# RomanBresson/KAGNN

Hardware: AMD Instinct MI355X
Metric: edges/sec KAN-GIN fwd+bwd, hidden=64 grid=5, 1M-node synthetic; HBM % peak (higher is better)
Workload: dtype f32 (fp16 hi/lo split operands, fp32 accumulate)

## Files before the change

### kagnn_amd/csrc/kan_sparse_fwd.hip

```cpp
#include "split_common.h"

namespace kagnn {

typedef _Float16 f16x16 __attribute__((ext_vector_type(16)));

constexpr int kSpCF = 64;
constexpr int kSpOutBlk = 64;
constexpr int kSpOutBlkWide = 128;
constexpr int kSpSteps = kSpCF / 4;
__host__ __device__ inline size_t sparse_fwd_chunk_bytes(int OT) {
    return (size_t)kSpSteps * OT * 2 * 2048 + (size_t)(kSpCF / 16) * OT * 2 * 1024;
}

bool kan_sparse_fwd_ok(int in, int out, int G, int K) { return K == 3 && G + K <= 16; }
__host__ __device__ inline int sp_sh(int C) { return C > 8 ? 1 : 0; }

static size_t sp_chunks_bytes(int inv, int ob) { return (size_t)cdiv(inv, kSpCF) * sparse_fwd_chunk_bytes(cdiv(ob, 32)); }
static size_t sp_blk_bytes(int in, int inv, int ob) { return kHdrBytes + sp_chunks_bytes(inv, ob) + (((size_t)ob * in * 4 + 255) & ~(size_t)255); }
static bool sp_wide_enabled() {
    static const bool on = [] { const char* e = getenv("KAGNN_FWD_WIDE"); return !(e && e[0] == '0'); }();
    return on;
}
static int sp_out_blk(int inv , int out) {
    return (sp_wide_enabled() && out % kSpOutBlkWide == 0 && inv > 32) ? kSpOutBlkWide : kSpOutBlk;
// ... 334 lines not shown
                    for (int st = 1; st < AEP; st <<= 1)
#pragma unroll
                        for (int k = 0; k < AEP; k += 2 * st) {
                            acc[g][h][k].x += acc[g][h][k + st].x; acc[g][h][k].y += acc[g][h][k + st].y;
                            acc[g][h][k].z += acc[g][h][k + st].z; acc[g][h][k].w += acc[g][h][k + st].w;
                        }
                    o[h] = make_float4(fmaf(sw, self[g][h].x, acc[g][h][0].x), fmaf(sw, self[g][h].y, acc[g][h][0].y),
                                       fmaf(sw, self[g][h].z, acc[g][h][0].z), fmaf(sw, self[g][h].w, acc[g][h][0].w));
                }
            }
            const int f0 = kg * HF + 8 * g;
            if (l0[g]) *reinterpret_cast<float4*>(ag.h0 + row * ag.ldh + f0) = o[0];
            if (l1[g]) *reinterpret_cast<float4*>(ag.h0 + row * ag.ldh + f0 + 4) = o[1];
            if (!l0[g]) o[0] = make_float4(0.f, 0.f, 0.f, 0.f);
            if (!l1[g]) o[1] = make_float4(0.f, 0.f, 0.f, 0.f);
            xa[g][0] = o[0].x; xa[g][1] = o[0].y; xa[g][2] = o[0].z; xa[g][3] = o[0].w;
            xa[g][4] = o[1].x; xa[g][5] = o[1].y; xa[g][6] = o[1].z; xa[g][7] = o[1].w;
        }
    };
    auto place1 = [&](const u32x4& e, unsigned h0, unsigned h1, unsigned l0, unsigned l1, unsigned& hi0, unsigned& hi1,
                      unsigned& lo0, unsigned& lo1) {
        hi0 = __builtin_amdgcn_perm(h1, h0, e[0]); hi1 = __builtin_amdgcn_perm(h1, h0, e[1]);
        lo0 = __builtin_amdgcn_perm(l1, l0, e[0]); lo1 = __builtin_amdgcn_perm(l1, l0, e[1]);
    };

    const int ng_live = HF / 8;
    (void)ng_live;
    float mom_n = 0.0f;
    float* s_momw = reinterpret_cast<float*>(s_w + BUF_BYTES) + wave * (OT * 64);
    if constexpr (MOM) {
#pragma unroll
        for (int t = 0; t < OT; ++t) s_momw[64 * t + lane] = 0.0f;
    }
    float xn[8];
    float xa[AGG >= 0 ? AGRP : 1][8];
    if constexpr (AGG >= 0) {
        gather_tile((long)blockIdx.x * ROWS, xa);
#pragma unroll
        for (int j = 0; j < 8; ++j) xn[j] = xa[0][j];
    } else load8((long)blockIdx.x * ROWS, ch_begin, 0, xn);
    for (long tile = blockIdx.x; tile * ROWS < N; tile += gridDim.x) {
        const long row0 = tile * ROWS + wave * 32;
        f32x16 acc[OT], acc_b[MERGED ? 1 : OT];
#pragma unroll
        for (int t = 0; t < OT; ++t)
#pragma unroll
            for (int i = 0; i < 16; ++i) { acc[t][i] = 0.0f; if constexpr (!MERGED) acc_b[t][i] = 0.0f; }

        for (int ch = ch_begin; ch < ch_end; ++ch) {
#pragma unroll
            for (int g = 0; g < NG; ++g) {
                if (g >= ng_live) continue;
                const int q = g / GPP, gq = g % GPP;
                const unsigned char* hb = s_w + (q & 1) * HALF_BYTES;
                if (!resident && gq == 0) {
                    lds_dma_wait();
                    __syncthreads();
#ifndef KAGNN_ABLATE_FWD_NO_REFILL
                    if (q + 1 < PPC) dma_half(ch, q + 1);
                    else if (ch + 1 < ch_end) dma_half(ch + 1, 0);
                    else if ((tile + gridDim.x) * ROWS < N) dma_half(ch_begin, 0);
#endif
                }
                float xv[8];
#pragma unroll
                for (int j = 0; j < 8; ++j) xv[j] = xn[j];
                if constexpr (AGG >= 0) {
                    if (g + 1 < ng_live) {
#pragma unroll
                        for (int j = 0; j < 8; ++j) xn[j] = xa[AGRP - 1][j];
                    } else {
                        gather_tile((tile + gridDim.x) * ROWS, xa);
#pragma unroll
                        for (int j = 0; j < 8; ++j) xn[j] = xa[0][j];
                    }
                } else if (g + 1 < ng_live) load8(tile * ROWS, ch, g + 1, xn);
                else if (ch + 1 < ch_end) load8(tile * ROWS, ch + 1, 0, xn);
                else load8((tile + gridDim.x) * ROWS, ch_begin, 0, xn);

                u32x4 ahi, alo, bw[4 * OT];
                int aidx;
                auto prep_reads = [&](int s, u32x4& e0, u32x4& e1, float& u0, float& u1, u32x4 (&w)[4 * OT]) {
                    unsigned o0, o1;
                    frag3_index<false>(xv[2 * s], f3geo, u0, o0);
                    if constexpr (SH) { u1 = u0; o1 = o0 + 512u; }
                    else frag3_index<false>(xv[2 * s + 1], f3geo, u1, o1);
                    e0 = *reinterpret_cast<const u32x4*>(reinterpret_cast<const unsigned char*>(s_tbl) + o0);
                    e1 = *reinterpret_cast<const u32x4*>(reinterpret_cast<const unsigned char*>(s_tbl) + o1);
                    if constexpr (MERGED) return;
                    const unsigned char* wp = hb + (size_t)((4 * gq + s) * OT) * 2 * 2048 + lane * 16;
#pragma unroll
                    for (int i = 0; i < 2 * OT; ++i) {
                        if (HALF && (i & 1)) continue;
                        w[2 * i] = *reinterpret_cast<const u32x4*>(wp + i * 2048);
                        w[2 * i + 1] = *reinterpret_cast<const u32x4*>(wp + i * 2048 + 1024);
                    }
                };
                auto read_w = [&](int s, u32x4 (&w)[4 * OT]) {
                    const unsigned char* wp = hb + (size_t)((4 * gq + s) * OT) * 2 * 2048 + lane * 16;
#pragma unroll
                    for (int i = 0; i < 2 * OT; ++i) {
                        w[2 * i] = *reinterpret_cast<const u32x4*>(wp + i * 2048);
                        w[2 * i + 1] = *reinterpret_cast<const u32x4*>(wp + i * 2048 + 1024);
                    }
                };
                auto build = [&](int s, const u32x4& e0, const u32x4& e1, float u0, float u1, u32x4& hi, u32x4& lo, int& idx) {
                    unsigned a0, a1, a2, a3, b0 = 0, b1 = 0, b2 = 0, b3 = 0, h0, h1, l0, l1;
#ifdef KAGNN_ABLATE_FWD_NO_EXPAND
                    hi = u32x4{__float_as_uint(u0), __float_as_uint(u1), e0[0], e1[0]};
                    lo = u32x4{e0[1], e1[1], __float_as_uint(u1), __float_as_uint(u0)};
                    idx = (int)(e0[2] | (e1[2] << 8));
// ... 120 lines not shown
                }
                if constexpr (!MERGED) {
                if (!big) {

                    const unsigned char* wp = hb + HALF_SPL + (size_t)(gq * OT) * 2 * 1024 + lane * 16;
#pragma unroll
                    for (int t = 0; t < OT; ++t) {
                        f32x16& ab = MERGED ? acc[t] : acc_b[MERGED ? 0 : t];
                        const u32x4 wh = *reinterpret_cast<const u32x4*>(wp + (t * 2 + 0) * 1024);
                        ab = mfma_f16(sh_hi, wh, ab);
                        if constexpr (!HALF) {
                            const u32x4 wl = *reinterpret_cast<const u32x4*>(wp + (t * 2 + 1) * 1024);
                            ab = mfma_f16(sh_hi, wl, ab);
                            ab = mfma_f16(sh_lo, wh, ab);
                        }
                    }
                } else {
                    const int f0 = ch * CF + kg * HF + 8 * g;
#pragma unroll
                    for (int j = 0; j < 8; ++j) {
#pragma unroll
                        for (int t = 0; t < OT; ++t) {
                            const int o = 32 * t + r;
                            const int fr = SH ? (f0 + j) >> 1 : f0 + j;
                            const float w = (o < out && fr < in && !(SH && (j & 1))) ? base_w[(long)o * in + fr] : 0.0f;
                            f32x16& ab = MERGED ? acc[t] : acc_b[MERGED ? 0 : t];
                            ab = __builtin_amdgcn_mfma_f32_32x32x2f32(sv[j] * (MERGED ? 0.0009765625f : 0.0625f), w * wsc16, ab, 0, 0, 0);
                        }
                    }
                }
                }
            }
        }
        const GBuf yb = gbuf_at(y, N, ldy, out, tile * ROWS);
        const long rows_here = min(32L, N - row0);
        const float mom_nt = (float)max(rows_here, 1L), mom_rnt = __builtin_amdgcn_rcpf(mom_nt);
        const float mom_w = mom_nt * __builtin_amdgcn_rcpf(mom_n + mom_nt), mom_nw = mom_n * mom_w;
#pragma unroll
        for (int t = 0; t < OT; ++t) {
            const int col = 32 * t + r;
            const unsigned base = (unsigned)(wave * 32 + 4 * kg) * ldy4 + col * 4;
            float v[16];
#pragma unroll
            for (int i = 0; i < 16; ++i) v[i] = MERGED ? acc[t][i] * post : fmaf(acc[t][i], post, acc_b[MERGED ? 0 : t][i] * post_b);
            if (col < out) {
#pragma unroll
                for (int i = 0; i < 16; ++i)
                    gst_s(yb, base, (unsigned)((i & 3) + 8 * (i >> 2)) * ldy4, v[i]);
            }
            if constexpr (MOM) {
                float sm = 0.0f, q = 0.0f, mt;
                if (rows_here >= 32) {
#pragma unroll
                    for (int i = 0; i < 16; ++i) sm += v[i];
                    sm += __shfl_xor(sm, 32);
                    mt = sm * mom_rnt;
#pragma unroll
                    for (int i = 0; i < 16; ++i) { const float d = v[i] - mt; q = fmaf(d, d, q); }
                } else {
#pragma unroll
                    for (int i = 0; i < 16; ++i) sm += (4 * kg + (i & 3) + 8 * (i >> 2) < rows_here) ? v[i] : 0.0f;
                    sm += __shfl_xor(sm, 32);
                    mt = sm * mom_rnt;
#pragma unroll
                    for (int i = 0; i < 16; ++i) {
                        const float d = (4 * kg + (i & 3) + 8 * (i >> 2) < rows_here) ? v[i] - mt : 0.0f;
                        q = fmaf(d, d, q);
// ... 373 lines not shown
```

### kagnn_amd/csrc/kan_split_bwd.hip

```cpp
#include <type_traits>
#include "split_common.h"

namespace kagnn {

int kan_dw_reduce(const float* slab, long NS, long per_slab, float* gcat, hipStream_t st);

int kan_dw_unpack(const float* gcat, int in, int out, int C, long inP, long outP, const float* sw,
                  const float* sc, float* g_bw, float* g_sw, float* g_sc, hipStream_t st);


bool kan_split_dx_ok(int in, int out, int G, int K) { return K >= 0 && K <= 4 && G + K <= 16; }
static inline int vshift(int C) { return C > 8 ? 1 : 0; }

static size_t dx_blk_bytes(int inv , int ob) {
    return kHdrBytes + (size_t)cdiv(inv, 16) * kCTmax * dx_q2(ob) * 2 * 1024;
}
bool kan_dx_w2_ok(int in, int out, int C, int K) { return K == 3 && C > 8 && C <= 16 && out <= kOutBlk; }
static int dx_inv(int in, int out, int C, int K) { return kan_dx_w2_ok(in, out, C, K) ? 32 * cdiv(in, 16) : (in << vshift(C)); }

size_t kan_split_pack_dx_bytes(int in, int out, int C, int K) {
    return (size_t)cdiv(out, kOutBlk) * dx_blk_bytes(dx_inv(in, out, C, K), min(out, kOutBlk));
}

__global__ void split_pack_dx_kernel(const float* __restrict__ bw, const float* __restrict__ sw,
// ... 86 lines not shown
        const unsigned char* src = gw + (size_t)ft0 * FT_BYTES;
        const int nblk = nft * (FT_BYTES / 1024);
        if constexpr (HALF) {
            for (int blk = 2 * wave; blk < nblk; blk += 16)
                lds_dma_1k(src + (size_t)blk * 1024 + lane * 16, __builtin_amdgcn_readfirstlane(lds_w + blk * 1024));
        } else
        for (int blk = wave; blk < nblk; blk += 8)
            lds_dma_1k(src + (size_t)blk * 1024 + lane * 16, __builtin_amdgcn_readfirstlane(lds_w + blk * 1024));
        lds_dma_wait();
    };
    const int ft_begin = blockIdx.y * ft_per_block, ft_end = min(FT, ft_begin + ft_per_block);
    if (resident) stage(ft_begin, ft_end - ft_begin);
    __syncthreads();
    const bool pingpong = (PP == 2) && resident;
    SplineGeom geom{}; FastGeom fgeo{};
    const int li = lane & 15, kg = lane >> 4;
    const int win = li & sh;
    float ca[8] = {};
    if constexpr (K == 0) {
        float c0[8], c1[8];
        rbf_centers(rb, c0, 0); rbf_centers(rb, c1, sh);
#pragma unroll
        for (int g = 0; g < 8; ++g) ca[g] = win ? c1[g] : c0[g];
    }
    if constexpr (K > 0) { geom = geom_from_knots(s_knots, nknots); fgeo = fast_geom(s_knots, nknots); }
    const bool ln_on = (K == 0) && rb.ln_w != nullptr;
    const bool al4 = ((ldgy & 3) == 0) && ((reinterpret_cast<uintptr_t>(gy) & 15) == 0);
    const unsigned ldx4 = (unsigned)ldx * 4u, ldgy4 = (unsigned)ldgy * 4u, ldgx4 = (unsigned)ldgx * gxes;
    const unsigned gy_ro = (unsigned)(wave * 32 + li) * ldgy4;
    const unsigned x_rb = (unsigned)(wave * 32 + 4 * kg) * ldx4;
    const unsigned gx_rb = (unsigned)(wave * 32 + 4 * kg) * ldgx4;
    const unsigned gz_rb = (unsigned)(wave * 32 + 4 * kg) * (unsigned)in * 4u;

    auto load_gy = [&](long tile, float (&raw)[2][Q2][8]) {
        const GBuf gyb = gbuf_at(gy, N, ldgy, out, tile * 256);
#pragma unroll
        for (int rt = 0; rt < 2; ++rt) {
            const unsigned ro = gy_ro + kg * 32;
            const unsigned so = (unsigned)(16 * rt) * ldgy4;
#pragma unroll
            for (int q = 0; q < Q2; ++q) {
                if (al4 && 32 * Q2 == out) {
                    gld4_s(gyb, ro, so + 128 * q, raw[rt][q]);
                    gld4_s(gyb, ro, so + 128 * q + 16, raw[rt][q] + 4);
                } else if (al4 && (out & 7) == 0) {
                    const unsigned rq = gy_ro + (unsigned)min(32 * q + 8 * kg, out - 8) * 4u;
                    gld4_s(gyb, rq, so, raw[rt][q]);
                    gld4_s(gyb, rq, so + 16, raw[rt][q] + 4);
                } else {
                    const int o0 = 32 * q + 8 * kg;
#pragma unroll
                    for (int j = 0; j < 8; ++j) raw[rt][q][j] = gld_s(gyb, gy_ro + min(o0 + j, out - 1) * 4, so);
                }
            }
        }
        if constexpr (BNB) {
            const GBuf yb = gbuf_at(bnb.y, N, bnb.ldy, out, tile * 256), ob = gbuf_at(bnb.gy_out, N, bnb.ldo, out, tile * 256);
            const unsigned ldy4 = (unsigned)bnb.ldy * 4u, ldo4 = (unsigned)bnb.ldo * 4u;
            const unsigned yro = (unsigned)(wave * 32 + li) * ldy4 + kg * 32, oro = (unsigned)(wave * 32 + li) * ldo4 + kg * 32;
#pragma unroll
            for (int q = 0; q < Q2; ++q) {
                float cm[8], cA[8], cB[8], cC[8];
                const float* t0 = bnb.tab + 32 * q + 8 * kg;
#pragma unroll
                for (int h = 0; h < 2; ++h) {
                    const float4 a = *reinterpret_cast<const float4*>(t0 + 4 * h), b = *reinterpret_cast<const float4*>(t0 + bnb.ldt + 4 * h);
                    const float4 c = *reinterpret_cast<const float4*>(t0 + 2 * bnb.ldt + 4 * h), d = *reinterpret_cast<const float4*>(t0 + 3 * bnb.ldt + 4 * h);
                    cm[4 * h] = a.x; cm[4 * h + 1] = a.y; cm[4 * h + 2] = a.z; cm[4 * h + 3] = a.w;
                    cA[4 * h] = b.x; cA[4 * h + 1] = b.y; cA[4 * h + 2] = b.z; cA[4 * h + 3] = b.w;
                    cB[4 * h] = c.x; cB[4 * h + 1] = c.y; cB[4 * h + 2] = c.z; cB[4 * h + 3] = c.w;
                    cC[4 * h] = d.x; cC[4 * h + 1] = d.y; cC[4 * h + 2] = d.z; cC[4 * h + 3] = d.w;
                }
#pragma unroll
                for (int rt = 0; rt < 2; ++rt) {
                    float yv[8];
                    gld4_s(yb, yro, (unsigned)(16 * rt) * ldy4 + 128 * q, yv);
                    gld4_s(yb, yro, (unsigned)(16 * rt) * ldy4 + 128 * q + 16, yv + 4);
#pragma unroll
                    for (int j = 0; j < 8; ++j) raw[rt][q][j] = bn_bwd_value(raw[rt][q][j], yv[j], cm[j], cA[j], cB[j], cC[j]);
                    if (blockIdx.y == 0) {
                        gst4_s(ob, oro, (unsigned)(16 * rt) * ldo4 + 128 * q, raw[rt][q]);
                        gst4_s(ob, oro, (unsigned)(16 * rt) * ldo4 + 128 * q + 16, raw[rt][q] + 4);
                    }
                }
            }
        }
    };
    u32x4 ahi[2][Q2], alo[2][Q2];
    float rinv[2][4];
    auto split_gy = [&](const float (&raw)[2][Q2][8]) {
#pragma unroll
        for (int rt = 0; rt < 2; ++rt) {
            float mx = 0.0f;
#pragma unroll
            for (int q = 0; q < Q2; ++q)
#pragma unroll
                for (int j = 0; j < 8; ++j) mx = fmaxf(mx, fabsf(raw[rt][q][j]));
            mx = fmaxf(mx, __shfl_xor(mx, 16));
            mx = fmaxf(mx, __shfl_xor(mx, 32));
            const int rexp = exp_for_max(mx);
            const float sc = ldexpf(1.0f, 10 - rexp);
#pragma unroll
            for (int q = 0; q < Q2; ++q) {
                float v[8];
#pragma unroll
                for (int j = 0; j < 8; ++j) v[j] = raw[rt][q][j] * sc;
                if constexpr (HALF) round_f16x2(v, ahi[rt][q]);
                else split_f16x2_asm(v, ahi[rt][q], alo[rt][q]);
            }
            const float mine = ldexpf(1.0f, e_w + rexp - 10);
#pragma unroll
            for (int reg = 0; reg < 4; ++reg) rinv[rt][reg] = __shfl(mine, 4 * kg + reg);
        }
    };
    float mu[2][4], rs[2][4];
    auto load_stats = [&](long tile) {
        if (ln_on) {
            const long row0 = tile * 256 + wave * 32;
#pragma unroll
            for (int rt = 0; rt < 2; ++rt)
#pragma unroll
                for (int reg = 0; reg < 4; ++reg) {
                    const long rc = min(row0 + 16 * rt + 4 * kg + reg, N - 1);
                    mu[rt][reg] = rb.stats[2 * rc]; rs[rt][reg] = rb.stats[2 * rc + 1];
                }
        }
    };

    float* s_stat = reinterpret_cast<float*>(s_w + (size_t)(ft_end - ft_begin) * FT_BYTES) + wave * 128;
    if constexpr (XST) { s_stat[lane] = 0.0f; s_stat[64 + lane] = 0.0f; }
    float graw[2][Q2][8];
    long tile = blockIdx.x;
    if (!XST && tile * 256 >= N) return;
    if (!XST || tile * 256 < N) {
    load_gy(tile, graw);
    load_stats(tile);
    split_gy(graw);
    if (PP >= 1 && (tile + gridDim.x) * 256 < N) load_gy(tile + gridDim.x, graw);
    }
    if (pingpong && wave >= 4) __builtin_amdgcn_s_barrier();

    for (; tile * 256 < N; tile += gridDim.x) {
        const bool more = (tile + gridDim.x) * 256 < N;
        if (PP == 0 && tile != (long)blockIdx.x) {
            load_gy(tile, graw);
            load_stats(tile);
            split_gy(graw);
        }
        const GBuf gzb = gbuf_at(rb.gz, N, in, in, tile * 256);
        const GBuf xb = gbuf_at(x, N, ldx, in, tile * 256), gxb = gbuf_at_es(gx, N, ldgx, in, tile * 256, (int)gxes);

        for (int ft = ft_begin; ft < ft_end; ++ft) {
            if (!resident) {
                __syncthreads();
                stage(ft, 1);
                __syncthreads();
            }
            const unsigned char* wft = s_w + (size_t)(resident ? ft - ft_begin : 0) * FT_BYTES + lane * 16;
            const int f = 16 * ft + li;
            const int fr = f >> sh;
            const unsigned fcol = (unsigned)min(fr, in - 1) * 4u;
            const unsigned gx_ro = gx_rb + (unsigned)min(fr, in - 1) * gxes, gz_ro = gz_rb + fcol;
            float gam = 1.0f, bet = 0.0f;
            if (ln_on) { gam = rb.ln_w[min(fr, in - 1)]; bet = rb.ln_b[min(fr, in - 1)]; }
            float xa = 1.0f, xs = 0.0f;
            if constexpr (XAFF) { xa = rb.x_affine[min(fr, in - 1)]; xs = rb.x_affine[in + min(fr, in - 1)]; }
            float st_m = 0.0f, st_q = 0.0f, st_g = 0.0f, st_gx = 0.0f;
            if constexpr (XST) { st_m = rb.st_mean[min(fr, in - 1)]; st_q = rb.st_rstd[min(fr, in - 1)]; }
            float xq[2][4];
#pragma unroll
            for (int rt = 0; rt < 2; ++rt)
#pragma unroll
                for (int reg = 0; reg < 4; ++reg) {
                    xq[rt][reg] = gld_s(xb, x_rb + fcol, (unsigned)(16 * rt + reg) * ldx4);
                }
            f32x4 D[kCTmax][2];
#pragma unroll
            for (int c = 0; c < kCTmax; ++c) { D[c][0] = f32x4{0.f, 0.f, 0.f, 0.f}; D[c][1] = f32x4{0.f, 0.f, 0.f, 0.f}; }
            {
                constexpr int NGRP = kCTmax * Q2;
#ifndef KAGNN_DX_LDS_DEPTH
#define KAGNN_DX_LDS_DEPTH 1
#endif
// ... 76 lines not shown
#pragma unroll
                    for (int c = 0; c < kCTmax - 1; ++c) d[c] = D[c][rt][reg];
                    float bar;
                    if constexpr (K == 3) {
                        const int mm = m - 8 * win;
                        const unsigned* be = s_btbl + kBarrelDw * min((unsigned)mm, 15u);
                        const u32x4 sel = *reinterpret_cast<const u32x4*>(be);
                        const uint2 rot = *reinterpret_cast<const uint2*>(be + 4);
                        bar = barrel_dot3(d, sel, rot.x, rot.y, dN) * (0.5f * fgeo.inv_h);
                    } else {
                        bar = barrel_dot<K>(d, m - 8 * win, dN);
                    }
                    float s = fmaf(D[kCTmax - 1][rt][reg], silu_gradf(xv), bar) * rinv[rt][reg];
                    if (sh) s += __shfl_xor(s, 1);
                    if constexpr (XST) {
                        st_g += s;
                        st_gx = fmaf(s, (xq[rt][reg] - st_m) * st_q, st_gx);
                    }
                    if (f < inv && win == 0) {
                        const unsigned so_x = (unsigned)(16 * rt + reg) * ldgx4;
                        if (ACC) s += gld_s(gxb, gx_ro, so_x);
                        if constexpr (GX16) gst16_s(gxb, gx_ro, so_x, s);
                        else gst_s(gxb, gx_ro, so_x, s);
                    }
                    }
                }
            }
            if constexpr (XST) {
                st_g += __shfl_xor(st_g, 16); st_gx += __shfl_xor(st_gx, 16);
                st_g += __shfl_xor(st_g, 32); st_gx += __shfl_xor(st_gx, 32);
                if (kg == 0 && f < in) { s_stat[f] += st_g; s_stat[64 + f] += st_gx; }
            }
            if (PP >= 1 && ft + 1 == ft_end && more) {
                load_stats(tile + gridDim.x);
                split_gy(graw);
                if ((tile + 2 * (long)gridDim.x) * 256 < N) load_gy(tile + 2 * (long)gridDim.x, graw);
            }
            if (pingpong) __builtin_amdgcn_s_barrier();
        }
    }
    if (pingpong && wave < 4) __builtin_amdgcn_s_barrier();
    if constexpr (XST) {
        __syncthreads();
        if (tid < 128) {
            const float* base = reinterpret_cast<const float*>(s_w + (size_t)(ft_end - ft_begin) * FT_BYTES);
            float a = 0.0f;
#pragma unroll
            for (int w8 = 0; w8 < 8; ++w8) a += base[w8 * 128 + tid];
            const int stat = tid >> 6, col = tid & 63;
            if (col < in) rb.st_partial[((long)blockIdx.x * 2 + stat) * in + col] = a;
        }
    }
}

template <int K, int Q2, bool GEN, int PP, bool GX16 = false, bool BNB = false, bool XAFF = false, bool XST = false, bool HALF = false>
static int launch_dx_pp(const float* x, long ldx, const float* gy, long ldgy, long N, int in, int out, int C,
                        const float* knots, int nknots, const unsigned char* pack, float* gx, long ldgx,
                        const RbfArgs& rb, int accumulate, hipStream_t st, const BnBack& bnb = BnBack{}) {
    if constexpr (!HALF && K == 3 && !GEN && Q2 <= 2 && PP != 2) {
        if (g_half_products)
            return launch_dx_pp<K, Q2, GEN, PP, GX16, BNB, XAFF, XST, true>(x, ldx, gy, ldgy, N, in, out, C, knots, nknots, pack, gx, ldgx, rb, accumulate, st, bnb);
    }
    const int sh = vshift(C), FT = cdiv(in << sh, 16);
    const size_t ft_bytes = (size_t)kCTmax * Q2 * 2 * 1024;
    const size_t budget = 160 * 1024 - kLdsHdr;
    const long row_blocks = cdiv(N, 256);
    int splits = row_blocks >= 128 ? 1 : (int)min((long)FT, 256 / row_blocks);
    const int fpb = cdiv(FT, splits);
    splits = cdiv(FT, fpb);
// ... 574 lines not shown
            if (!step(raw)) break;
        if (n0 < rend) rescale(raw);
    }
    if constexpr (K == 0) {
        if (bias_on) {
#pragma unroll
            for (int t = 0; t < NTO; ++t) {
                float v = bsum[t];
                v += __shfl_xor(v, 16);
                v += __shfl_xor(v, 32);
                const long o = 16 * NTO * oc + 16 * t + li;
                if (kg == 0 && o < outP) rb.colpart[s * outP + o] = v;
            }
        }
    }
    const float undo = ldexpf(1.0f, T - 20), undo_b = ldexpf(1.0f, T - 14);
#pragma unroll
    for (int t = 0; t < NTO; ++t) {
        const long o = 16 * NTO * oc + 16 * t + li;
#pragma unroll
        for (int reg = 0; reg < 4; ++reg) {
            const long fl = 64 * fg + 16 * tile + 4 * kg + reg;
            if (fl < inP && o < outP) {
#pragma unroll
                for (int c = 0; c < kCTmax - 1; ++c)
                    if (c < C) slab[((s * (C + 1) + c) * inP + fl) * outP + o] = D[c][t][reg] * undo;
                slab[((s * (C + 1) + C) * inP + fl) * outP + o] = Dh[t][reg] * undo_b;
            }
        }
    }
}
#undef Dh

constexpr int kDwShVecs = 18;
constexpr int kDwShChunkBytes = kDwShVecs * 64 * 16;
constexpr int kDwShFlagOff = 2304;
constexpr size_t kDwShLds = kLdsHdr + 8 * (size_t)kDwShChunkBytes;

template <int K, int SH>
__global__ __launch_bounds__(256, 1) void kan_split_dw_shared_kernel(
    const float* __restrict__ x, long ldx, const float* __restrict__ gy, long ldgy, long N, int in,
    int out, int C, const float* __restrict__ knots_g, int nknots, int OC, long rows_per_block,
    long inP, long outP, float* __restrict__ slab, RbfArgs rb) {
    constexpr int NTO = 4, TPW = 4 / SH;
    extern __shared__ __attribute__((aligned(16))) unsigned char smem[];
    float* s_knots = reinterpret_cast<float*>(smem);
    unsigned* s_tbl = reinterpret_cast<unsigned*>(smem + 256);
    int* s_flag = reinterpret_cast<int*>(smem + kDwShFlagOff);
    const int tid = threadIdx.x, wave = tid >> 6, lane = tid & 63;
    if (K > 0 && tid < nknots) s_knots[tid] = knots_g[tid];
    if (K > 0) build_perm_table(s_tbl, tid);
    __syncthreads();
    FastGeom fgeo{};
    const int li = lane & 15, kg = lane >> 4;
    const int wave_u = __builtin_amdgcn_readfirstlane(wave);
    const int tl = wave_u / SH, ocl = wave_u % SH;
    const int OCG = OC / SH;
    const int tile = (blockIdx.y / OCG) * TPW + tl;
    const int oc = (blockIdx.y % OCG) * SH + ocl;
    const int f = 16 * tile + li;
    float ca[8] = {};
    if constexpr (K == 0) rbf_centers(rb, ca, 0);
    if constexpr (K > 0) fgeo = fast_geom(s_knots, nknots);
    const bool ln_on = (K == 0) && rb.ln_w != nullptr;
    const long s = blockIdx.x;
    const long rbeg = blockIdx.x * rows_per_block;
// ... 577 lines not shown
            static unsigned long long seen_##KK##_##SS = 0; \
            if (auto first_use_ = first_use_on_this_device(seen_##KK##_##SS)) \
                KAGNN_HIP(hipFuncSetAttribute((const void*)kan_split_dw_shared_kernel<KK, SS>, hipFuncAttributeMaxDynamicSharedMemorySize, (int)kDwShLds)); \
            kan_split_dw_shared_kernel<KK, SS><<<grid, 256, kDwShLds, st>>>(x, ldx, gy, ldgy, N, in, out, Ck, knots, nk, p.OC, p.rpw, p.inP, p.outP, slab, rb); } while (0)
        if (K == 0) { if (SHn == 4) LS(0, 4); else LS(0, 2); }
        else        { if (SHn == 4) LS(3, 4); else LS(3, 2); }
#undef LS
        KAGNN_LAUNCH_CHECK();
        return dw_reduce_unpack(slab, p.NS, in, out, C, p.inP, p.outP, sw, sc, g_bw, g_sw, g_sc, st);
    }
    const bool half = g_half_products && K == 3 && !sh;
#define LH(RR, NN, XX) kan_split_dw_kernel<3, false, RR, NN, XX, true><<<grid, 256, 0, st>>>(ARGS, 0)
#define LN(KK) if (p.rs == 4) kan_split_dw_kernel<KK, false, 4><<<grid, 256, 0, st>>>(ARGS, 0); \
               else if (p.rs == 2) kan_split_dw_kernel<KK, false, 2><<<grid, 256, 0, st>>>(ARGS, 0); \
               else if (nto == 3) kan_split_dw_kernel<KK, false, 1, 3><<<grid, 256, 0, st>>>(ARGS, 0); \
               else if (nto == 2) kan_split_dw_kernel<KK, false, 1, 2><<<grid, 256, 0, st>>>(ARGS, 0); \
               else if (nto == 1) kan_split_dw_kernel<KK, false, 1, 1><<<grid, 256, 0, st>>>(ARGS, 0); \
               else { L(KK); }
    if (rb.x_affine) {
        if (K != 3 || sh || p.rs != 1) return fail(KAGNN_ERR_UNSUPPORTED, "%s: an input affine needs a cubic layer with <= 8 coefficients and more than 32 inputs", "kan_split_dw");
        if (half) { if (nto == 3) LH(1, 3, true); else if (nto == 2) LH(1, 2, true); else if (nto == 1) LH(1, 1, true); else LH(1, 4, true); }
        else if (nto == 3) kan_split_dw_kernel<3, false, 1, 3, true><<<grid, 256, 0, st>>>(ARGS, 0);
        else if (nto == 2) kan_split_dw_kernel<3, false, 1, 2, true><<<grid, 256, 0, st>>>(ARGS, 0);
        else if (nto == 1) kan_split_dw_kernel<3, false, 1, 1, true><<<grid, 256, 0, st>>>(ARGS, 0);
        else kan_split_dw_kernel<3, false, 1, 4, true><<<grid, 256, 0, st>>>(ARGS, 0);
    } else if (half) {
        if (p.rs == 4) LH(4, 4, false); else if (p.rs == 2) LH(2, 4, false);
        else if (nto == 3) LH(1, 3, false); else if (nto == 2) LH(1, 2, false); else if (nto == 1) LH(1, 1, false); else LH(1, 4, false);
    } else
    switch (K) {
        case 0: LN(0); break;
        case 1: L(1); break;
        case 2: L(2); break;
        case 3: LN(3); break;
        case 4: L(4); break;
        default: return fail(KAGNN_ERR_UNSUPPORTED, "%s: spline_order must be 1..4", "kan_split_dw");
    }
#undef L
#undef LN
#undef LH
#undef ARGS
    KAGNN_LAUNCH_CHECK();
    if (!sh) {
        return dw_reduce_unpack(slab, p.NS, in, out, C, p.inP, p.outP, sw, sc, g_bw, g_sw, g_sc, st);
    }
    { int rc = kan_dw_reduce(slab, p.NS, p.per, gcat, st); if (rc) return rc; }
    if (sh) {
        kan_dw_unpack_v_kernel<<<cdiv((long)in * out, 256), 256, 0, st>>>(gcat, in, out, C, p.inP, p.outP, sw, sc, g_bw, g_sw, g_sc);
        KAGNN_LAUNCH_CHECK();
        return KAGNN_OK;
    }
    return kan_dw_unpack(gcat, in, out, C, p.inP, p.outP, sw, sc, g_bw, g_sw, g_sc, st);
}

int kan_split_dw(const float* x, long ldx, const float* gy, long ldgy, long N, const float* knots, int in,
                 int out, int G, int K, const float* sw, const float* sc, float* g_bw, float* g_sw,
                 float* g_sc, float* ws, size_t ws_bytes, hipStream_t st, const float* x_affine) {
    RbfArgs rb{};
    rb.x_affine = x_affine;
    if (x_affine && (kan_dw_w2_ok(in, out, G + K, K) || out > 64))
        return fail(KAGNN_ERR_UNSUPPORTED, "%s: an input affine needs a cubic layer with <= 8 coefficients and <= 64 outputs", "kan_split_dw");
    return kan_split_dw_any(x, ldx, gy, ldgy, N, knots, in, out, G, K, sw, sc, g_bw, g_sw, g_sc, ws, ws_bytes, rb, st);
}

}
```

### kagnn_amd/csrc/split_common.h

```cpp
#pragma once
#include "common.h"

namespace kagnn {

typedef __bf16 bf16x8 __attribute__((ext_vector_type(8)));
typedef float f32x2 __attribute__((ext_vector_type(2)));
__device__ __forceinline__ f32x2 fma2(f32x2 a, f32x2 b, f32x2 c) { return __builtin_elementwise_fma(a, b, c); }
__device__ __forceinline__ f32x2 splat2(float v) { return f32x2{v, v}; }

constexpr int kHdrBytes = 256;
constexpr int kLdsHdr = 2560;
constexpr unsigned kWinBytes = 512;
constexpr float kAScale = 1024.0f;
constexpr int kOutBlk = 128;

__device__ __forceinline__ float wcat_s(const float* bw, const float* sw, const float* sc, int in,
                                        int out, int C, int o, int f, int c) {
    if (o >= out || f >= in || c > C) return 0.0f;
    if (c == C) return bw ? bw[(long)o * in + f] : 0.0f;
    float w = sw[((long)o * in + f) * C + c];
    return sc ? w * sc[(long)o * in + f] : w;
}

__device__ __forceinline__ float wcat_v(const float* bw, const float* sw, const float* sc, int in,
// ... 316 lines not shown
    ahi[2] = __builtin_amdgcn_perm(h1, h0, sel[2]); ahi[3] = __builtin_amdgcn_perm(h1, h0, sel[3]);
    alo[0] = __builtin_amdgcn_perm(l1, l0, sel[0]); alo[1] = __builtin_amdgcn_perm(l1, l0, sel[1]);
    alo[2] = __builtin_amdgcn_perm(l1, l0, sel[2]); alo[3] = __builtin_amdgcn_perm(l1, l0, sel[3]);
    if constexpr (K >= 4) {
        const float n4 = N[K >= 4 ? 4 : 0] * kAScale;
        const unsigned h2 = pk_f16_rtz(n4, 0.0f);
        const unsigned l2 = pk_f16_rtz(sub_f16lo(n4, h2), 0.0f);
        const u32x4 fix = *reinterpret_cast<const u32x4*>(reinterpret_cast<const unsigned char*>(tbl) + kFixBytes + woff + 16 * t);
#pragma unroll
        for (int q = 0; q < 4; ++q) {
            ahi[q] = __builtin_amdgcn_perm(h2, ahi[q], fix[q]);
            alo[q] = __builtin_amdgcn_perm(l2, alo[q], fix[q]);
        }
    }
}

__device__ __forceinline__ void make_spline_frag3(float x, const unsigned* __restrict__ tbl,
                                                  const FastGeom& g, u32x4& ahi, u32x4& alo,
                                                  unsigned woff = 0) {
    int m; float u; bool inside;
    fast_span(x, g, m, u, inside);
    float N[4];
    cubic_bases(u, inside ? (kAScale / 6.0f) : 0.0f, N);
    const unsigned h0 = pk_f16_rtz(N[0], N[1]), h1 = pk_f16_rtz(N[2], N[3]);
    const unsigned l0 = pk_f16_rtz(sub_f16lo(N[0], h0), sub_f16hi(N[1], h0));
    const unsigned l1 = pk_f16_rtz(sub_f16lo(N[2], h1), sub_f16hi(N[3], h1));
    const u32x4 sel = *reinterpret_cast<const u32x4*>(reinterpret_cast<const unsigned char*>(tbl) + woff + 16 * (m + 1));
    ahi[0] = __builtin_amdgcn_perm(h1, h0, sel[0]); ahi[1] = __builtin_amdgcn_perm(h1, h0, sel[1]);
    ahi[2] = __builtin_amdgcn_perm(h1, h0, sel[2]); ahi[3] = __builtin_amdgcn_perm(h1, h0, sel[3]);
    alo[0] = __builtin_amdgcn_perm(l1, l0, sel[0]); alo[1] = __builtin_amdgcn_perm(l1, l0, sel[1]);
    alo[2] = __builtin_amdgcn_perm(l1, l0, sel[2]); alo[3] = __builtin_amdgcn_perm(l1, l0, sel[3]);
}

__device__ __forceinline__ void make_spline_frag3_pair(float x0, float x1, const unsigned* __restrict__ tbl,
                                                       const FastGeom& g, u32x4& ahi0, u32x4& alo0,
                                                       u32x4& ahi1, u32x4& alo1, unsigned woff = 0) {
    const f32x2 x = {x0, x1};
#ifdef KAGNN_ABLATE_SHARED_EXPANSION
    const int m0 = (int)(__float_as_uint(x0) & 7u), m1 = (int)(__float_as_uint(x1) & 7u);
    const f32x2 N0 = x, N1 = x, N2 = x, N3 = x;
    (void)g;
#else
    const f32x2 t = fma2(x, splat2(g.inv_h), splat2(g.c0));
    const f32x2 tf = {fminf(fmaxf(floorf(t.x), 0.0f), g.last_span), fminf(fmaxf(floorf(t.y), 0.0f), g.last_span)};
    const int m0 = (int)tf.x, m1 = (int)tf.y;
    const f32x2 u = t - tf;
    const f32x2 w6 = {(x0 >= g.k_first && x0 < g.k_last) ? kAScale / 6.0f : 0.0f,
                      (x1 >= g.k_first && x1 < g.k_last) ? kAScale / 6.0f : 0.0f};
    const f32x2 u2 = u * u, om = splat2(1.0f) - u, uw = u * w6, ow = om * w6;
    const f32x2 N0 = ow * (om * om);
    const f32x2 N3 = uw * u2;
    const f32x2 N1 = fma2(uw, fma2(u, splat2(3.0f), splat2(-6.0f)) * u, splat2(4.0f) * w6);
    const f32x2 N2 = fma2(uw, fma2(fma2(u, splat2(-3.0f), splat2(3.0f)), u, splat2(3.0f)), w6);
#endif
    {
        const unsigned h0 = pk_f16_rtz(N0.x, N1.x), h1 = pk_f16_rtz(N2.x, N3.x);
        const unsigned l0 = pk_f16_rtz(sub_f16lo(N0.x, h0), sub_f16hi(N1.x, h0));
        const unsigned l1 = pk_f16_rtz(sub_f16lo(N2.x, h1), sub_f16hi(N3.x, h1));
        const u32x4 sel = *reinterpret_cast<const u32x4*>(reinterpret_cast<const unsigned char*>(tbl) + woff + 16 * (m0 + 1));
        frag3_place_fwd(sel, h0, h1, l0, l1, ahi0, alo0);
    }
    {
        const unsigned h0 = pk_f16_rtz(N0.y, N1.y), h1 = pk_f16_rtz(N2.y, N3.y);
        const unsigned l0 = pk_f16_rtz(sub_f16lo(N0.y, h0), sub_f16hi(N1.y, h0));
        const unsigned l1 = pk_f16_rtz(sub_f16lo(N2.y, h1), sub_f16hi(N3.y, h1));
        const u32x4 sel = *reinterpret_cast<const u32x4*>(reinterpret_cast<const unsigned char*>(tbl) + woff + 16 * (m1 + 1));
        frag3_place_fwd(sel, h0, h1, l0, l1, ahi1, alo1);
    }
}

__device__ __forceinline__ void make_spline_frag3_pair_h(float x0, float x1, const unsigned* __restrict__ tbl,
                                                         const FastGeom& g, u32x4& ahi0, u32x4& ahi1, unsigned woff = 0) {
    const f32x2 x = {x0, x1};
    const f32x2 t = fma2(x, splat2(g.inv_h), splat2(g.c0));
    const f32x2 tf = {fminf(fmaxf(floorf(t.x), 0.0f), g.last_span), fminf(fmaxf(floorf(t.y), 0.0f), g.last_span)};
    const int m0 = (int)tf.x, m1 = (int)tf.y;
    const f32x2 u = t - tf;
    const f32x2 w6 = {(x0 >= g.k_first && x0 < g.k_last) ? kAScale / 6.0f : 0.0f,
                      (x1 >= g.k_first && x1 < g.k_last) ? kAScale / 6.0f : 0.0f};
    const f32x2 u2 = u * u, om = splat2(1.0f) - u, uw = u * w6, ow = om * w6;
    const f32x2 N0 = ow * (om * om);
    const f32x2 N3 = uw * u2;
    const f32x2 N1 = fma2(uw, fma2(u, splat2(3.0f), splat2(-6.0f)) * u, splat2(4.0f) * w6);
    const f32x2 N2 = fma2(uw, fma2(fma2(u, splat2(-3.0f), splat2(3.0f)), u, splat2(3.0f)), w6);
    {
        const unsigned h0 = pk_f16_rne(N0.x, N1.x), h1 = pk_f16_rne(N2.x, N3.x);
        const u32x4 sel = *reinterpret_cast<const u32x4*>(reinterpret_cast<const unsigned char*>(tbl) + woff + 16 * (m0 + 1));
        ahi0[0] = __builtin_amdgcn_perm(h1, h0, sel[0]); ahi0[1] = __builtin_amdgcn_perm(h1, h0, sel[1]);
        ahi0[2] = __builtin_amdgcn_perm(h1, h0, sel[2]); ahi0[3] = __builtin_amdgcn_perm(h1, h0, sel[3]);
    }
    {
        const unsigned h0 = pk_f16_rne(N0.y, N1.y), h1 = pk_f16_rne(N2.y, N3.y);
        const u32x4 sel = *reinterpret_cast<const u32x4*>(reinterpret_cast<const unsigned char*>(tbl) + woff + 16 * (m1 + 1));
        ahi1[0] = __builtin_amdgcn_perm(h1, h0, sel[0]); ahi1[1] = __builtin_amdgcn_perm(h1, h0, sel[1]);
        ahi1[2] = __builtin_amdgcn_perm(h1, h0, sel[2]); ahi1[3] = __builtin_amdgcn_perm(h1, h0, sel[3]);
    }
}

struct Frag3Geom { float inv_h, c1; };
__device__ __forceinline__ Frag3Geom frag3_geom(const float* knots, int nknots) {
// ... 197 lines not shown
```

Measured before the change: 4.488 billion.

## Rebalance tail tiles at 32-row granularity across blocks in sparse fwd and split bwd

```diff
diff --git a/kagnn_amd/csrc/kan_sparse_fwd.hip b/kagnn_amd/csrc/kan_sparse_fwd.hip
--- a/kagnn_amd/csrc/kan_sparse_fwd.hip
+++ b/kagnn_amd/csrc/kan_sparse_fwd.hip
@@ -390,6 +390,23 @@
 #pragma unroll
         for (int t = 0; t < OT; ++t) s_momw[64 * t + lane] = 0.0f;
     }
+    constexpr bool GRAN = OT == 2 && !SH && !MOM && !NARROW && AGG < 0 && !PARTS && !HALF;
+    const long t0_stride = (long)gridDim.x * ROWS;
+    long gran_from = N, gran_t0 = N;
+    if constexpr (GRAN) {
+        if (resident && gridDim.y == 1) {
+            const long full = ((N + ROWS - 1) / ROWS) / gridDim.x;
+            const int wave_s = __builtin_amdgcn_readfirstlane(tid >> 6);
+            gran_from = full * t0_stride;
+            const long g = blockIdx.x + (long)wave_s * gridDim.x;
+            if (gran_from + g * 32 < N) gran_t0 = gran_from + (g - wave_s) * 32;
+        }
+    }
+    auto next_t0 = [&](long t0) -> long {
+        const long n = t0 + t0_stride;
+        if constexpr (GRAN) return t0 >= gran_from ? N : (n >= gran_from ? gran_t0 : n);
+        return n;
+    };
     float xn[8];
     float xa[AGG >= 0 ? AGRP : 1][8];
     if constexpr (AGG >= 0) {
@@ -397,8 +414,8 @@
 #pragma unroll
         for (int j = 0; j < 8; ++j) xn[j] = xa[0][j];
     } else load8((long)blockIdx.x * ROWS, ch_begin, 0, xn);
-    for (long tile = blockIdx.x; tile * ROWS < N; tile += gridDim.x) {
-        const long row0 = tile * ROWS + wave * 32;
+    for (long t0 = (long)blockIdx.x * ROWS; t0 < N; t0 = next_t0(t0)) {
+        const long row0 = t0 + wave * 32;
         f32x16 acc[OT], acc_b[MERGED ? 1 : OT];
 #pragma unroll
         for (int t = 0; t < OT; ++t)
@@ -417,7 +434,7 @@
 #ifndef KAGNN_ABLATE_FWD_NO_REFILL
                     if (q + 1 < PPC) dma_half(ch, q + 1);
                     else if (ch + 1 < ch_end) dma_half(ch + 1, 0);
-                    else if ((tile + gridDim.x) * ROWS < N) dma_half(ch_begin, 0);
+                    else if (next_t0(t0) < N) dma_half(ch_begin, 0);
 #endif
                 }
                 float xv[8];
@@ -428,13 +445,13 @@
 #pragma unroll
                         for (int j = 0; j < 8; ++j) xn[j] = xa[AGRP - 1][j];
                     } else {
-                        gather_tile((tile + gridDim.x) * ROWS, xa);
+                        gather_tile(next_t0(t0), xa);
 #pragma unroll
                         for (int j = 0; j < 8; ++j) xn[j] = xa[0][j];
                     }
-                } else if (g + 1 < ng_live) load8(tile * ROWS, ch, g + 1, xn);
-                else if (ch + 1 < ch_end) load8(tile * ROWS, ch + 1, 0, xn);
-                else load8((tile + gridDim.x) * ROWS, ch_begin, 0, xn);
+                } else if (g + 1 < ng_live) load8(t0, ch, g + 1, xn);
+                else if (ch + 1 < ch_end) load8(t0, ch + 1, 0, xn);
+                else load8(next_t0(t0), ch_begin, 0, xn);
 
                 u32x4 ahi, alo, bw[4 * OT];
                 int aidx;
@@ -621,7 +638,7 @@
                 }
             }
         }
-        const GBuf yb = gbuf_at(y, N, ldy, out, tile * ROWS);
+        const GBuf yb = gbuf_at(y, N, ldy, out, t0);
         const long rows_here = min(32L, N - row0);
         const float mom_nt = (float)max(rows_here, 1L), mom_rnt = __builtin_amdgcn_rcpf(mom_nt);
         const float mom_w = mom_nt * __builtin_amdgcn_rcpf(mom_n + mom_nt), mom_nw = mom_n * mom_w;
diff --git a/kagnn_amd/csrc/kan_split_bwd.hip b/kagnn_amd/csrc/kan_split_bwd.hip
--- a/kagnn_amd/csrc/kan_split_bwd.hip
+++ b/kagnn_amd/csrc/kan_split_bwd.hip
@@ -142,8 +142,8 @@
     const unsigned gx_rb = (unsigned)(wave * 32 + 4 * kg) * ldgx4;
     const unsigned gz_rb = (unsigned)(wave * 32 + 4 * kg) * (unsigned)in * 4u;
 
-    auto load_gy = [&](long tile, float (&raw)[2][Q2][8]) {
-        const GBuf gyb = gbuf_at(gy, N, ldgy, out, tile * 256);
+    auto load_gy = [&](long t0 , float (&raw)[2][Q2][8]) {
+        const GBuf gyb = gbuf_at(gy, N, ldgy, out, t0);
 #pragma unroll
         for (int rt = 0; rt < 2; ++rt) {
             const unsigned ro = gy_ro + kg * 32;
@@ -165,7 +165,7 @@
             }
         }
         if constexpr (BNB) {
-            const GBuf yb = gbuf_at(bnb.y, N, bnb.ldy, out, tile * 256), ob = gbuf_at(bnb.gy_out, N, bnb.ldo, out, tile * 256);
+            const GBuf yb = gbuf_at(bnb.y, N, bnb.ldy, out, t0), ob = gbuf_at(bnb.gy_out, N, bnb.ldo, out, t0);
             const unsigned ldy4 = (unsigned)bnb.ldy * 4u, ldo4 = (unsigned)bnb.ldo * 4u;
             const unsigned yro = (unsigned)(wave * 32 + li) * ldy4 + kg * 32, oro = (unsigned)(wave * 32 + li) * ldo4 + kg * 32;
 #pragma unroll
@@ -224,9 +224,9 @@
         }
     };
     float mu[2][4], rs[2][4];
-    auto load_stats = [&](long tile) {
+    auto load_stats = [&](long t0) {
         if (ln_on) {
-            const long row0 = tile * 256 + wave * 32;
+            const long row0 = t0 + wave * 32;
 #pragma unroll
             for (int rt = 0; rt < 2; ++rt)
 #pragma unroll
@@ -240,25 +240,43 @@
     float* s_stat = reinterpret_cast<float*>(s_w + (size_t)(ft_end - ft_begin) * FT_BYTES) + wave * 128;
     if constexpr (XST) { s_stat[lane] = 0.0f; s_stat[64 + lane] = 0.0f; }
     float graw[2][Q2][8];
-    long tile = blockIdx.x;
-    if (!XST && tile * 256 >= N) return;
-    if (!XST || tile * 256 < N) {
-    load_gy(tile, graw);
-    load_stats(tile);
+    constexpr bool GRAN = K == 3 && Q2 == 2 && !GEN && PP == 1 && !GX16 && !BNB && !XAFF && !XST && !HALF;
+    const long t0_stride = (long)gridDim.x * 256;
+    long gran_from = N, gran_t0 = N;
+    if constexpr (GRAN) {
+        if (resident && gridDim.y == 1) {
+            const long full = ((N + 255) / 256) / gridDim.x;
+            const int wave_s = __builtin_amdgcn_readfirstlane(tid >> 6);
+            gran_from = full * t0_stride;
+            const long g = blockIdx.x + (long)wave_s * gridDim.x;
+            if (gran_from + g * 32 < N) gran_t0 = gran_from + (g - wave_s) * 32;
+        }
+    }
+    auto next_t0 = [&](long t0) -> long {
+        const long n = t0 + t0_stride;
+        if constexpr (GRAN) return t0 >= gran_from ? N : (n >= gran_from ? gran_t0 : n);
+        return n;
+    };
+    long t0 = (long)blockIdx.x * 256;
+    if (!XST && t0 >= N) return;
+    if (!XST || t0 < N) {
+    load_gy(t0, graw);
+    load_stats(t0);
     split_gy(graw);
-    if (PP >= 1 && (tile + gridDim.x) * 256 < N) load_gy(tile + gridDim.x, graw);
+    if (PP >= 1 && next_t0(t0) < N) load_gy(next_t0(t0), graw);
     }
     if (pingpong && wave >= 4) __builtin_amdgcn_s_barrier();
 
-    for (; tile * 256 < N; tile += gridDim.x) {
-        const bool more = (tile + gridDim.x) * 256 < N;
-        if (PP == 0 && tile != (long)blockIdx.x) {
-            load_gy(tile, graw);
-            load_stats(tile);
+    for (; t0 < N; t0 = next_t0(t0)) {
+        const long t1 = next_t0(t0);
+        const bool more = t1 < N;
+        if (PP == 0 && t0 != (long)blockIdx.x * 256) {
+            load_gy(t0, graw);
+            load_stats(t0);
             split_gy(graw);
         }
-        const GBuf gzb = gbuf_at(rb.gz, N, in, in, tile * 256);
-        const GBuf xb = gbuf_at(x, N, ldx, in, tile * 256), gxb = gbuf_at_es(gx, N, ldgx, in, tile * 256, (int)gxes);
+        const GBuf gzb = gbuf_at(rb.gz, N, in, in, t0);
+        const GBuf xb = gbuf_at(x, N, ldx, in, t0), gxb = gbuf_at_es(gx, N, ldgx, in, t0, (int)gxes);
 
         for (int ft = ft_begin; ft < ft_end; ++ft) {
             if (!resident) {
@@ -401,9 +419,9 @@
                 if (kg == 0 && f < in) { s_stat[f] += st_g; s_stat[64 + f] += st_gx; }
             }
             if (PP >= 1 && ft + 1 == ft_end && more) {
-                load_stats(tile + gridDim.x);
+                load_stats(t1);
                 split_gy(graw);
-                if ((tile + 2 * (long)gridDim.x) * 256 < N) load_gy(tile + 2 * (long)gridDim.x, graw);
+                if (next_t0(t1) < N) load_gy(next_t0(t1), graw);
             }
             if (pingpong) __builtin_amdgcn_s_barrier();
         }
```

New measurement: 4.524 billion (median of 6 runs). About the same (+0.8%).

## Split cubic dW coefficient columns across two wave groups in a 512-thread kernel

Applied to the files above, without the earlier changes.

```diff
diff --git a/kagnn_amd/csrc/kan_split_bwd.hip b/kagnn_amd/csrc/kan_split_bwd.hip
--- a/kagnn_amd/csrc/kan_split_bwd.hip
+++ b/kagnn_amd/csrc/kan_split_bwd.hip
@@ -1044,6 +1044,180 @@
 }
 #undef Dh
 
+template <int PART>
+__device__ __forceinline__ void dw_ps_body(const float* __restrict__ x, long ldx, const float* __restrict__ gy, long ldgy,
+                                           long N, int in, int out, int C, const unsigned* __restrict__ s_tbl,
+                                           const FastGeom& fgeo, int fg, int oc, int tile, int lane, long rows_per_block,
+                                           long inP, long outP, float* __restrict__ slab) {
+    constexpr int NTO = 4, NP = PART ? 5 : 4;
+    const int li = lane & 15, kg = lane >> 4;
+    const int f = 64 * fg + 16 * tile + li;
+    const long s = blockIdx.x;
+    const long rbeg = blockIdx.x * rows_per_block;
+    const long rend = min(N, (blockIdx.x + 1L) * rows_per_block);
+
+    f32x4 D[NP][NTO];
+#define Dh D[NP - 1]
+#pragma unroll
+    for (int c = 0; c < NP; ++c)
+#pragma unroll
+        for (int t = 0; t < NTO; ++t) D[c][t] = f32x4{0.f, 0.f, 0.f, 0.f};
+
+    const GBuf xb = gbuf_at(x, rend, ldx, in, rbeg), gyb = gbuf_at(gy, rend, ldgy, out, rbeg);
+    const unsigned ldx4 = (unsigned)ldx * 4u, ldgy4 = (unsigned)ldgy * 4u;
+    unsigned xo = (unsigned)(8 * kg) * ldx4 + (unsigned)min(f, in - 1) * 4u, gvo[NTO];
+#pragma unroll
+    for (int t = 0; t < NTO; ++t) gvo[t] = (unsigned)(8 * kg) * ldgy4 + (unsigned)min(16 * NTO * oc + 16 * t + li, out - 1) * 4u;
+    auto load_raw = [&](DwRaw<NTO>& r) {
+#pragma unroll
+        for (int j = 0; j < 8; ++j) r.x[j] = gld_s(xb, xo, (unsigned)j * ldx4);
+#pragma unroll
+        for (int j = 0; j < 8; ++j)
+#pragma unroll
+            for (int t = 0; t < NTO; ++t) r.g[t][j] = gld_s(gyb, gvo[t], (unsigned)j * ldgy4);
+        xo += 32u * ldx4;
+#pragma unroll
+        for (int t = 0; t < NTO; ++t) gvo[t] += 32u * ldgy4;
+    };
+    auto chunk_exp = [&](const DwRaw<NTO>& r) -> int {
+        float mx = 0.0f;
+#pragma unroll
+        for (int t = 0; t < NTO; ++t)
+#pragma unroll
+            for (int j = 0; j < 8; ++j) mx = fmaxf(mx, fabsf(r.g[t][j]));
+        return exp_for_max(wave_max_nonneg(mx));
+    };
+
+    int T;
+    auto step = [&](DwRaw<NTO>& raw) -> bool {
+        u32x2 rh[8], rl[8];
+#pragma unroll
+        for (int j = 0; j < 8; j += 2)
+            make_spline_frag3_pair_words<PART>(raw.x[j], raw.x[j + 1], s_tbl, fgeo, rh[j], rl[j], rh[j + 1], rl[j + 1]);
+        u32x4 sah, sal;
+        float sv[8];
+        bool base32 = false;
+        if constexpr (PART == 1) {
+            float smx = 0.0f;
+#pragma unroll
+            for (int j = 0; j < 8; j += 2) {
+                const f32x2 pr = silu16_pair(f32x2{raw.x[j], raw.x[j + 1]});
+                sv[j] = pr.x; sv[j + 1] = pr.y;
+                smx = fmaxf(fmaxf(smx, fabsf(pr.x)), fabsf(pr.y));
+            }
+            base32 = __any(!(smx < 60000.0f));
+            split_f16x2(sv, sah, sal);
+        }
+        if (chunk_exp(raw) > T) return false;
+        u32x4 bhi[NTO], blo[NTO];
+        const float gs = ldexpf(1.0f, 10 - T);
+#pragma unroll
+        for (int t = 0; t < NTO; ++t) {
+            float v[8];
+#pragma unroll
+            for (int j = 0; j < 8; j += 2) {
+                const f32x2 pr = f32x2{raw.g[t][j], raw.g[t][j + 1]} * splat2(gs);
+                v[j] = pr.x; v[j + 1] = pr.y;
+            }
+            split_f16x2(v, bhi[t], blo[t]);
+        }
+        if constexpr (PART == 1) {
+            if (base32) {
+                const float gs16 = gs * 16.0f;
+#pragma unroll
+                for (int j = 0; j < 8; ++j) {
+                    const float sj = sv[j] * 0.0625f;
+#pragma unroll
+                    for (int t = 0; t < NTO; ++t)
+                        Dh[t] = __builtin_amdgcn_mfma_f32_16x16x4f32(sj, raw.g[t][j] * gs16, Dh[t], 0, 0, 0);
+                }
+            }
+        }
+        load_raw(raw);
+#pragma unroll
+        for (int c = 0; c < 4; ++c) {
+            const int q = c >> 1;
+            const unsigned sel = (c & 1) ? 0x07060302u : 0x05040100u;
+            u32x4 ah, al;
+#pragma unroll
+            for (int p = 0; p < 4; ++p) {
+                ah[p] = __builtin_amdgcn_perm(rh[2 * p + 1][q], rh[2 * p][q], sel);
+                al[p] = __builtin_amdgcn_perm(rl[2 * p + 1][q], rl[2 * p][q], sel);
+            }
+#pragma unroll
+            for (int t = 0; t < NTO; ++t) D[c][t] = mfma16_f16(ah, bhi[t], D[c][t]);
+#pragma unroll
+            for (int t = 0; t < NTO; ++t) D[c][t] = mfma16_f16(ah, blo[t], D[c][t]);
+#pragma unroll
+            for (int t = 0; t < NTO; ++t) D[c][t] = mfma16_f16(al, bhi[t], D[c][t]);
+        }
+        if constexpr (PART == 1) {
+            if (!base32) {
+#pragma unroll
+                for (int t = 0; t < NTO; ++t) Dh[t] = mfma16_f16(sah, bhi[t], Dh[t]);
+#pragma unroll
+                for (int t = 0; t < NTO; ++t) Dh[t] = mfma16_f16(sah, blo[t], Dh[t]);
+#pragma unroll
+                for (int t = 0; t < NTO; ++t) Dh[t] = mfma16_f16(sal, bhi[t], Dh[t]);
+            }
+        }
+        return true;
+    };
+    auto rescale = [&](DwRaw<NTO>& raw) {
+        const int ex = chunk_exp(raw);
+        const float dn = ldexpf(1.0f, T - ex);
+#pragma unroll
+        for (int c = 0; c < NP; ++c)
+#pragma unroll
+            for (int t = 0; t < NTO; ++t) D[c][t] *= dn;
+        T = ex;
+    };
+    long n0 = rbeg;
+    DwRaw<NTO> raw;
+    load_raw(raw);
+    T = chunk_exp(raw);
+    while (n0 < rend) {
+        for (; n0 < rend; n0 += 32)
+            if (!step(raw)) break;
+        if (n0 < rend) rescale(raw);
+    }
+    const float undo = ldexpf(1.0f, T - 20), undo_b = ldexpf(1.0f, T - 14);
+#pragma unroll
+    for (int t = 0; t < NTO; ++t) {
+        const long o = 16 * NTO * oc + 16 * t + li;
+#pragma unroll
+        for (int reg = 0; reg < 4; ++reg) {
+            const long fl = 64 * fg + 16 * tile + 4 * kg + reg;
+            if (fl < inP && o < outP) {
+#pragma unroll
+                for (int c = 0; c < 4; ++c)
+                    if (4 * PART + c < C) slab[((s * (C + 1) + 4 * PART + c) * inP + fl) * outP + o] = D[c][t][reg] * undo;
+                if constexpr (PART == 1) slab[((s * (C + 1) + C) * inP + fl) * outP + o] = Dh[t][reg] * undo_b;
+            }
+        }
+    }
+#undef Dh
+}
+
+__global__ __launch_bounds__(512) void kan_split_dw_ps_kernel(
+    const float* __restrict__ x, long ldx, const float* __restrict__ gy, long ldgy, long N, int in,
+    int out, int C, const float* __restrict__ knots_g, int nknots, int OC, long rows_per_block,
+    long inP, long outP, float* __restrict__ slab) {
+    __shared__ __attribute__((aligned(16))) unsigned char smem[kLdsHdr];
+    float* s_knots = reinterpret_cast<float*>(smem);
+    unsigned* s_tbl = reinterpret_cast<unsigned*>(smem + 256);
+    const int tid = threadIdx.x, wave = tid >> 6, lane = tid & 63;
+    if (tid < nknots) s_knots[tid] = knots_g[tid];
+    build_perm_table(s_tbl, tid);
+    __syncthreads();
+    const FastGeom fgeo = fast_geom(s_knots, nknots);
+    const int fg = blockIdx.y / OC, oc = blockIdx.y % OC;
+    const int wave_u = __builtin_amdgcn_readfirstlane(wave);
+    const int tile = wave_u & 3;
+    if (wave_u < 4) dw_ps_body<0>(x, ldx, gy, ldgy, N, in, out, C, s_tbl, fgeo, fg, oc, tile, lane, rows_per_block, inP, outP, slab);
+    else            dw_ps_body<1>(x, ldx, gy, ldgy, N, in, out, C, s_tbl, fgeo, fg, oc, tile, lane, rows_per_block, inP, outP, slab);
+}
+
 constexpr int kDwShVecs = 18;
 constexpr int kDwShChunkBytes = kDwShVecs * 64 * 16;
 constexpr int kDwShFlagOff = 2304;
@@ -1687,7 +1861,11 @@
         case 0: LN(0); break;
         case 1: L(1); break;
         case 2: L(2); break;
-        case 3: LN(3); break;
+        case 3:
+            if (!sh && p.rs == 1 && nto == 4)
+                kan_split_dw_ps_kernel<<<grid, 512, 0, st>>>(x, ldx, gy, ldgy, N, in, out, Ck, knots, nk, p.OC, p.rpw, p.inP, p.outP, slab);
+            else { LN(3); }
+            break;
         case 4: L(4); break;
         default: return fail(KAGNN_ERR_UNSUPPORTED, "%s: spline_order must be 1..4", "kan_split_dw");
     }
diff --git a/kagnn_amd/csrc/split_common.h b/kagnn_amd/csrc/split_common.h
--- a/kagnn_amd/csrc/split_common.h
+++ b/kagnn_amd/csrc/split_common.h
@@ -372,9 +372,8 @@
     alo[2] = __builtin_amdgcn_perm(l1, l0, sel[2]); alo[3] = __builtin_amdgcn_perm(l1, l0, sel[3]);
 }
 
-__device__ __forceinline__ void make_spline_frag3_pair(float x0, float x1, const unsigned* __restrict__ tbl,
-                                                       const FastGeom& g, u32x4& ahi0, u32x4& alo0,
-                                                       u32x4& ahi1, u32x4& alo1, unsigned woff = 0) {
+struct Frag3PairPayload { int m[2]; unsigned h0[2], h1[2], l0[2], l1[2]; };
+__device__ __forceinline__ Frag3PairPayload frag3_pair_payload(float x0, float x1, const FastGeom& g) {
     const f32x2 x = {x0, x1};
 #ifdef KAGNN_ABLATE_SHARED_EXPANSION
     const int m0 = (int)(__float_as_uint(x0) & 7u), m1 = (int)(__float_as_uint(x1) & 7u);
@@ -393,19 +392,47 @@
     const f32x2 N1 = fma2(uw, fma2(u, splat2(3.0f), splat2(-6.0f)) * u, splat2(4.0f) * w6);
     const f32x2 N2 = fma2(uw, fma2(fma2(u, splat2(-3.0f), splat2(3.0f)), u, splat2(3.0f)), w6);
 #endif
+    Frag3PairPayload p;
+    p.m[0] = m0; p.m[1] = m1;
+    p.h0[0] = pk_f16_rtz(N0.x, N1.x); p.h1[0] = pk_f16_rtz(N2.x, N3.x);
+    p.l0[0] = pk_f16_rtz(sub_f16lo(N0.x, p.h0[0]), sub_f16hi(N1.x, p.h0[0]));
+    p.l1[0] = pk_f16_rtz(sub_f16lo(N2.x, p.h1[0]), sub_f16hi(N3.x, p.h1[0]));
+    p.h0[1] = pk_f16_rtz(N0.y, N1.y); p.h1[1] = pk_f16_rtz(N2.y, N3.y);
+    p.l0[1] = pk_f16_rtz(sub_f16lo(N0.y, p.h0[1]), sub_f16hi(N1.y, p.h0[1]));
+    p.l1[1] = pk_f16_rtz(sub_f16lo(N2.y, p.h1[1]), sub_f16hi(N3.y, p.h1[1]));
+    return p;
+}
+__device__ __forceinline__ void make_spline_frag3_pair(float x0, float x1, const unsigned* __restrict__ tbl,
+                                                       const FastGeom& g, u32x4& ahi0, u32x4& alo0,
+                                                       u32x4& ahi1, u32x4& alo1, unsigned woff = 0) {
+    const Frag3PairPayload p = frag3_pair_payload(x0, x1, g);
     {
-        const unsigned h0 = pk_f16_rtz(N0.x, N1.x), h1 = pk_f16_rtz(N2.x, N3.x);
-        const unsigned l0 = pk_f16_rtz(sub_f16lo(N0.x, h0), sub_f16hi(N1.x, h0));
-        const unsigned l1 = pk_f16_rtz(sub_f16lo(N2.x, h1), sub_f16hi(N3.x, h1));
-        const u32x4 sel = *reinterpret_cast<const u32x4*>(reinterpret_cast<const unsigned char*>(tbl) + woff + 16 * (m0 + 1));
-        frag3_place_fwd(sel, h0, h1, l0, l1, ahi0, alo0);
+        const u32x4 sel = *reinterpret_cast<const u32x4*>(reinterpret_cast<const unsigned char*>(tbl) + woff + 16 * (p.m[0] + 1));
+        frag3_place_fwd(sel, p.h0[0], p.h1[0], p.l0[0], p.l1[0], ahi0, alo0);
     }
     {
-        const unsigned h0 = pk_f16_rtz(N0.y, N1.y), h1 = pk_f16_rtz(N2.y, N3.y);
-        const unsigned l0 = pk_f16_rtz(sub_f16lo(N0.y, h0), sub_f16hi(N1.y, h0));
-        const unsigned l1 = pk_f16_rtz(sub_f16lo(N2.y, h1), sub_f16hi(N3.y, h1));
-        const u32x4 sel = *reinterpret_cast<const u32x4*>(reinterpret_cast<const unsigned char*>(tbl) + woff + 16 * (m1 + 1));
-        frag3_place_fwd(sel, h0, h1, l0, l1, ahi1, alo1);
+        const u32x4 sel = *reinterpret_cast<const u32x4*>(reinterpret_cast<const unsigned char*>(tbl) + woff + 16 * (p.m[1] + 1));
+        frag3_place_fwd(sel, p.h0[1], p.h1[1], p.l0[1], p.l1[1], ahi1, alo1);
+    }
+}
+
+__device__ __forceinline__ void frag3_place_fwd_words(const u32x2& sel, unsigned h0, unsigned h1, unsigned l0,
+                                                      unsigned l1, u32x2& ahi, u32x2& alo) {
+    ahi[0] = __builtin_amdgcn_perm(h1, h0, sel[0]); ahi[1] = __builtin_amdgcn_perm(h1, h0, sel[1]);
+    alo[0] = __builtin_amdgcn_perm(l1, l0, sel[0]); alo[1] = __builtin_amdgcn_perm(l1, l0, sel[1]);
+}
+template <int WP>
+__device__ __forceinline__ void make_spline_frag3_pair_words(float x0, float x1, const unsigned* __restrict__ tbl,
+                                                             const FastGeom& g, u32x2& ahi0, u32x2& alo0,
+                                                             u32x2& ahi1, u32x2& alo1) {
+    const Frag3PairPayload p = frag3_pair_payload(x0, x1, g);
+    {
+        const u32x2 sel = *reinterpret_cast<const u32x2*>(reinterpret_cast<const unsigned char*>(tbl) + 8 * WP + 16 * (p.m[0] + 1));
+        frag3_place_fwd_words(sel, p.h0[0], p.h1[0], p.l0[0], p.l1[0], ahi0, alo0);
+    }
+    {
+        const u32x2 sel = *reinterpret_cast<const u32x2*>(reinterpret_cast<const unsigned char*>(tbl) + 8 * WP + 16 * (p.m[1] + 1));
+        frag3_place_fwd_words(sel, p.h0[1], p.h1[1], p.l0[1], p.l1[1], ahi1, alo1);
     }
 }
 
```

After: 4.243 billion before, 3.979 billion after. -6.2%, worse.
